# kserve/modelmesh

Hardware: AMD Instinct MI355X
Metric: placement decisions/sec at 100k models x 10k pods; p99 decision latency (higher is better)
Workload: dtype i64; 1 GPU; C3: 100000 models x 10000 pods, 8 load-target decision(s) per model per step = 800000 decisions per launch (SURVEY.md §8d synthetic fleet); streams=4, hw_queues=4, distinct_batches=6, issuers=1, library_submission_threads=0, resident_input_bytes=384000000

## Files before the change

modelmesh_amd/csrc/mmplace.hip:

```cpp
#include <hip/hip_runtime.h>
#include <dlfcn.h>
#include <rccl/rccl.h>
#include <rocprim/device/device_radix_sort.hpp>
#include <chrono>
#include <rocprim/device/device_merge_sort.hpp>
#include <rocprim/device/device_scan.hpp>

#include <algorithm>
#include <atomic>
#include <cstdarg>
#include <cstdio>
#include <cstdlib>
#include <cstring>
#include <map>
#include <memory>
#include <mutex>
#include <shared_mutex>
#include <thread>
#include <new>
#include <string>
#include <unordered_map>
#include <vector>

#include "../../include/mmplace.h"
// ... 23 lines not shown

thread_local std::string g_thread_err;

struct DevBuf {
    void *p = nullptr;
    size_t cap = 0;
    hipError_t ensure(size_t bytes)
    {
        if (bytes <= cap) return hipSuccess;
        if (p) (void)hipFree(p);
        p = nullptr;
        cap = 0;
        size_t want = std::max<size_t>(bytes, 256);
        want = (want + 255) & ~size_t(255);
        hipError_t e = hipMalloc(&p, want);
        if (e == hipSuccess) cap = want;
        return e;
    }
    void release()
    {
        if (p) (void)hipFree(p);
        p = nullptr;
        cap = 0;
    }
    template <class T>
    T *as() const { return reinterpret_cast<T *>(p); }
};

struct SnapBufs {
    DevBuf pods, lru, rem, cnt, rpm, orig, pos_of, elig, elig_nors, pref, has_pref, fullw, ge, pc, ph, nz, heads, bslots, bpm, bwin, bsurv, bpcs;
    DevBuf sel, rk;
    DevBuf amul;
    int32_t amul_w = 0;
    DevBuf memo, memo_cand, memo_rk;
    DevBuf lmemo;
    DevBuf ctpos;
    uint64_t types_gen = 0;
    int32_t n_bslots = 0;
    void release()
    {
        for (DevBuf *b : {&pods, &lru, &rem, &cnt, &rpm, &orig, &pos_of, &elig, &elig_nors, &pref, &has_pref, &fullw, &ge, &pc, &ph, &nz, &heads, &bslots, &bpm, &bwin, &bsurv, &bpcs, &ctpos, &sel, &rk, &amul, &memo, &memo_cand, &memo_rk, &lmemo})
            b->release();
    }
};

template <class SnapT>
SnapT snap_columns(const SnapBufs &B, int32_t P, int32_t W, int32_t T, bool any_rs, int64_t min_space)
{
    SnapT S{};
    S.P = P;
    S.W = W;
    S.T = T;
    S.any_rs = any_rs;
    S.min_space = min_space;
    S.lru = B.lru.as<int64_t>();
    S.rem = B.rem.as<int64_t>();
    S.cnt = B.cnt.as<int32_t>();
    S.rpm = B.rpm.as<int32_t>();
    S.orig = B.orig.as<int32_t>();
    S.pos_of = B.pos_of.as<int32_t>();
    S.elig = B.elig.as<uint64_t>();
    S.elig_nors = B.elig_nors.as<uint64_t>();
    S.pref = B.pref.as<uint64_t>();
    S.has_pref = B.has_pref.as<uint8_t>();
    S.fullw = B.fullw.as<uint64_t>();
    return S;
}

struct SnapSide {
    DevBuf d_allowed, d_has_allowed, stats_acc, d_pts, d_prohib, pstats, tstats, rmodels;
    DevBuf mtw;
    uint64_t types_gen = 0;
    bool rmodels_ok = false;
    std::vector<int32_t> pts_of;
// ... 1733 lines not shown
    HIP_TRY(c, B.elig_nors.ensure((size_t)T * Wc * 8));
    HIP_TRY(c, B.pref.ensure((size_t)T * Wc * 8));
    HIP_TRY(c, B.has_pref.ensure(T));
    HIP_TRY(c, B.fullw.ensure((size_t)Wc * 8));
    HIP_TRY(c, B.ge.ensure((size_t)kGeRows * Wc * 8));
    return MMP_OK;
}
int ensure_commit_scratch(mmp_ctx *c, SnapSide &N, int32_t T, int32_t W)
{
    HIP_TRY(c, c->occupancy.ensure((size_t)W * 64 * 4));
    HIP_TRY(c, c->flag.ensure(sizeof(int32_t)));
    HIP_TRY(c, N.stats_acc.ensure(sizeof(StatsAcc)));
    HIP_TRY(c, c->rs_bad.ensure((size_t)W * 64));
    HIP_TRY(c, c->rs_list.ensure(std::max<size_t>(c->replaced_rs.size(), 1) * 4));
    HIP_TRY(c, N.d_allowed.ensure(std::max<size_t>((size_t)T * W, 1) * 8));
    HIP_TRY(c, c->d_prefer.ensure(std::max<size_t>((size_t)T * W, 1) * 8));
    HIP_TRY(c, N.d_has_allowed.ensure(T));
    return MMP_OK;
}
int ensure_snapshot_buffers(mmp_ctx *c, SnapBufs &B, SnapSide &N, const CommitDims &D)
{
    const int32_t T = D.T, W = D.W;
    HIP_TRY(c, B.pods.ensure(std::max<size_t>(D.P, 1) * sizeof(mmp_pod_row)));
    if (const int rc = ensure_columns(c, B, T, W, W)) return rc;
    HIP_TRY(c, B.ctpos.ensure((size_t)(kGeRows + 1) * 4));
    HIP_TRY(c, B.pc.ensure((size_t)2 * T * (W + 1) * 4));
    HIP_TRY(c, B.nz.ensure((size_t)2 * T * (W + 1) * 4));
    HIP_TRY(c, B.ph.ensure((size_t)2 * T * (W + 1) * 8));
    if (D.have_sel) {
        HIP_TRY(c, B.sel.ensure(D.sel_bytes));
        HIP_TRY(c, B.rk.ensure(D.sel_bytes));
    }
    if (D.have_lmemo) HIP_TRY(c, B.lmemo.ensure((size_t)T * kLongLevels * sizeof(LongMemo)));
    HIP_TRY(c, B.memo.ensure((size_t)kWinLds * sizeof(TypeMemo)));
    HIP_TRY(c, B.memo_cand.ensure((size_t)kWinLds * kMemoCand * 4));
    HIP_TRY(c, B.memo_rk.ensure((size_t)kWinLds * kMemoCand * 2));
    HIP_TRY(c, B.heads.ensure(D.wins_bytes));
    HIP_TRY(c, B.bslots.ensure(kBSlots * sizeof(BSlot) + 16));
    HIP_TRY(c, B.bpm.ensure((size_t)kBSlots * W * 64 * 4));
    HIP_TRY(c, B.bwin.ensure(kBSlots * sizeof(BLaunch)));
    HIP_TRY(c, B.bsurv.ensure((size_t)kBSlots * kBClasses * W * 8));
    HIP_TRY(c, B.bpcs.ensure((size_t)kBSlots * kBClasses * (W + 1) * 4));
    HIP_TRY(c, c->rank.ensure(D.padded * 4));
    return ensure_commit_scratch(c, N, T, W);
}

void clear_commit_scratch(mmp_ctx *c, SnapBufs &B, const CommitDims &D, hipStream_t st)
{
    ZeroBatch zb(st);
    zb.add(c->rank.p, D.padded * 4);
    zb.add(c->occupancy.p, D.padded * 4);
    zb.add(c->flag.p, sizeof(int32_t));
    zb.add(B.bslots.p, kBSlots * sizeof(BSlot) + 16);
    zb.launch(st);
    hipLaunchKernelGGL(zero_tails_kernel, dim3(1), dim3(64), 0, st, B.lru.as<int64_t>(), B.rem.as<int64_t>(), B.cnt.as<int32_t>(),
                       B.rpm.as<int32_t>(), B.orig.as<int32_t>(), B.pos_of.as<int32_t>(), D.P, (int32_t)D.padded);
}

struct OrderCheck {
    bool sort_legal;
    int32_t n_present, n_nonfull;
};
OrderCheck check_placement_order(const std::vector<mmp_pod_row> &pods, int64_t min_space, int64_t churn2)
{
    bool versions_differ = false, full_low_lru = false, wide_count = false;
    OrderCheck oc{};
    for (const mmp_pod_row &r : pods) {
// ... 105 lines not shown
    }
    const size_t n_rs = c->replaced_rs.size();
    if (n_rs) HIP_TRY(c, hipMemcpyAsync(c->rs_list.p, c->replaced_rs.data(), n_rs * 4, hipMemcpyHostToDevice, st));
    in.init = StatsAcc{};
    in.init.global_lru = INT64_MAX;
    HIP_TRY(c, hipMemcpyAsync(N.stats_acc.p, &in.init, sizeof in.init, hipMemcpyHostToDevice, st));
    return MMP_OK;
}

int ensure_audit_multipliers(mmp_ctx *c, SnapBufs &B, int32_t W, hipStream_t st)
{
    if (B.amul_w == W) return MMP_OK;
    HIP_TRY(c, B.amul.ensure((size_t)W * 8));
    std::vector<uint64_t> am((size_t)W);
    for (int32_t w = 0; w < W; w++) am[(size_t)w] = audit_mul((uint64_t)w);
    HIP_TRY(c, hipMemcpyAsync(B.amul.p, am.data(), (size_t)W * 8, hipMemcpyHostToDevice, st));
    HIP_TRY(c, hipStreamSynchronize(st));
    B.amul_w = W;
    return MMP_OK;
}

Snap snap_of(const SnapBufs &B, const CommitDims &D)
{
    Snap S = snap_columns<Snap>(B, D.P, D.W, D.T, D.n_rs > 0, D.min_space);
    S.ge = B.ge.as<uint64_t>();
    S.pc = B.pc.as<int32_t>();
    S.nz = B.nz.as<int32_t>();
    S.ph = B.ph.as<uint64_t>();
    S.ctpos = D.P > 0 ? B.ctpos.as<int32_t>() : nullptr;
    S.amul = B.amul.as<uint64_t>();
    S.sel = D.P > 0 && D.have_sel ? B.sel.as<int32_t>() : nullptr;
    S.rk = D.P > 0 && D.have_sel ? B.rk.as<int32_t>() : nullptr;
    S.memo = B.memo.as<TypeMemo>();
    S.memo_cand = B.memo_cand.as<int32_t>();
    S.memo_rk = B.memo_rk.as<int16_t>();
    S.lmemo = D.have_lmemo ? B.lmemo.as<LongMemo>() : nullptr;
    return S;
}

int launch_rank(mmp_ctx *c, const mmp_pod_row *d_pods, int32_t P, int32_t p_lo, int32_t p_hi, bool slice, bool want_sort, bool sort_legal,
                int32_t *d_rank, hipStream_t st)
{
    const int64_t min_space = c->cfg.min_space_units, churn2 = churn2_of(c);
    if (want_sort && sort_legal && P >= kSampleMinPods && c->tune.rank_mode != 3)
        return rank_by_sampling(c, d_pods, P, min_space, churn2, p_lo, p_hi, d_rank, st);
    if (want_sort && sort_legal && P >= 2) {
        HIP_TRY(c, c->rk_rows.ensure((size_t)P * sizeof(RankRow)));
        HIP_TRY(c, c->rk_idx.ensure((size_t)P * sizeof(RankRow)));
        const PlacementRowLess less{churn2};
        size_t tmp_bytes = 0;
        HIP_TRY(c, rocprim::merge_sort(nullptr, tmp_bytes, c->rk_rows.as<RankRow>(), c->rk_idx.as<RankRow>(), (size_t)P, less, st));
        HIP_TRY(c, c->rk_tmp.ensure(std::max<size_t>(tmp_bytes, 16)));
        hipLaunchKernelGGL(rank_rows_kernel, dim3(div_up(P, 256)), dim3(256), 0, st, d_pods, P, min_space, c->rk_rows.as<RankRow>());
        HIP_TRY(c, rocprim::merge_sort(c->rk_tmp.p, tmp_bytes, c->rk_rows.as<RankRow>(), c->rk_idx.as<RankRow>(), (size_t)P, less, st));
        if (slice)
            hipLaunchKernelGGL(rank_from_order_range_kernel, dim3(div_up(P, 256)), dim3(256), 0, st, c->rk_idx.as<RankRow>(), P, p_lo, p_hi, d_rank);
        else
            hipLaunchKernelGGL(rank_from_order_kernel, dim3(div_up(P, 256)), dim3(256), 0, st, c->rk_idx.as<RankRow>(), P, d_rank);
        return MMP_OK;
    }
    const int pb = div_up(p_hi - p_lo, kRankBlock);
    const int slices = std::max(1, std::min(64, 2048 / pb));
    hipLaunchKernelGGL(rank_pods_kernel, dim3(pb, slices), dim3(kRankBlock), 0, st, d_pods, P, min_space, churn2, slices, p_lo, p_hi, d_rank);
    return MMP_OK;
}

// ... 35 lines not shown
    L1.nb_ge = div_up(kGeRows * W, 4);
    L1.nb_stats = std::min(div_up(P, 256), 512);
    L1.nb_pstats = N.n_pts > 0 ? std::min(div_up(P, 256), 64) : 0;
    return L1;
}
inline int32_t *n_bslots_dev(const SnapBufs &B) { return reinterpret_cast<int32_t *>(static_cast<char *>(B.bslots.p) + kBSlots * sizeof(BSlot)); }
CommitL2 make_commit_l2(const mmp_ctx *c, const SnapBufs &B, const SnapSide &N, const Snap &S)
{
    CommitL2 L2{};
    L2.S = S;
    L2.pods = B.pods.as<mmp_pod_row>();
    L2.wins = B.heads.as<TypeWin>();
    L2.slots = B.bslots.as<BSlot>();
    L2.n_slots = n_bslots_dev(B);
    L2.acc = N.stats_acc.as<StatsAcc>();
    L2.pstats = N.pstats.as<StatsAcc>();
    L2.NP = N.n_pts;
    L2.Tw = N.pts_tw;
    L2.prohib = N.d_prohib.as<uint64_t>();
    L2.has_allowed = c->n_types > 0 ? N.d_has_allowed.as<uint8_t>() : nullptr;
    L2.tstats = N.tstats.as<StatsAcc>();
    L2.nb_finish = div_up(std::max(N.n_pts, S.T), 64);
    return L2;
}
void launch_snapshot_tables(mmp_ctx *c, SnapBufs &B, SnapSide &N, const Snap &S, const CommitDims &D, hipStream_t st)
{
    const int32_t T = D.T, W = D.W;
    const CommitL1 L1 = make_commit_l1(c, B, N, D);
    hipLaunchKernelGGL(commit_level1_kernel, dim3(L1.nb_stats + L1.nb_pstats + 1 + L1.nb_masks + L1.nb_ge), dim3(256), 0, st, L1);
    const CommitL2 L2 = make_commit_l2(c, B, N, S);
    hipLaunchKernelGGL(commit_level2_kernel, dim3(4 * T + L2.nb_finish), dim3(64), 0, st, L2);
    hipLaunchKernelGGL(build_sel_memo_kernel, dim3((D.have_sel ? 2 * T * W : 0) + std::min(T, kWinLds) + (S.lmemo ? T : 0)), dim3(64), 0, st, S,
                       D.have_sel ? B.sel.as<int32_t>() : nullptr, D.have_sel ? B.rk.as<int32_t>() : nullptr, B.heads.as<TypeWin>(),
                       B.memo.as<TypeMemo>(), B.memo_cand.as<int32_t>(), B.memo_rk.as<int16_t>(), B.lmemo.as<LongMemo>());
    hipLaunchKernelGGL(prefix_min_rpm_kernel, dim3(kBSlots), dim3(64), 0, st, S, B.bslots.as<BSlot>(), n_bslots_dev(B), B.bpm.as<int32_t>(),
                       (int32_t)(W * 64));
    hipLaunchKernelGGL(build_bsurv_kernel, dim3(kBSlots), dim3(256), 0, st, S, B.bslots.as<BSlot>(), n_bslots_dev(B), B.bpm.as<int32_t>(),
                       (int32_t)(W * 64), B.bwin.as<BLaunch>(), B.bsurv.as<uint64_t>(), B.bpcs.as<int32_t>());
}
int clear_snapshot_tables(mmp_ctx *c, SnapBufs &B, const CommitDims &D, hipStream_t st)
{
    const size_t T = D.T, W = D.W;
    HIP_TRY(c, hipMemsetAsync(B.heads.p, 0, D.wins_bytes, st));
    HIP_TRY(c, hipMemsetAsync(B.memo.p, 0, (size_t)kWinLds * sizeof(TypeMemo), st));
    HIP_TRY(c, hipMemsetAsync(B.pc.p, 0, 2 * T * (W + 1) * 4, st));
    HIP_TRY(c, hipMemsetAsync(B.nz.p, 0, 2 * T * (W + 1) * 4, st));
    HIP_TRY(c, hipMemsetAsync(B.ph.p, 0, 2 * T * (W + 1) * 8, st));
    HIP_TRY(c, hipMemsetAsync(B.elig.p, 0, T * W * 8, st));
    HIP_TRY(c, hipMemsetAsync(B.elig_nors.p, 0, T * W * 8, st));
    HIP_TRY(c, hipMemsetAsync(B.pref.p, 0, T * W * 8, st));
    HIP_TRY(c, hipMemsetAsync(B.fullw.p, 0, W * 8, st));
    HIP_TRY(c, hipMemsetAsync(B.ge.p, 0, kGeRows * W * 8, st));
    return MMP_OK;
}


int stage_partitions(mmp_ctx *c, SnapSide &N, int32_t P, hipStream_t st)
{
    const int32_t T = std::max(c->n_types, 1), Tw = div_up(T, 64);
    N.pts_of.assign(P, -1);
    N.pts_prohib.clear();
    N.n_pts = 0;
    N.pts_tw = Tw;
    if (c->n_types > 0) {
        if (!c->sig_valid || (int32_t)c->sig_of.size() != P) {
            std::map<std::vector<uint64_t>, int32_t> intern;
            std::vector<uint64_t> sig(Tw);
            const int32_t Wf = c->types_w;
            c->sig_of.assign(P, 0);
            c->sig_rows.clear();
            for (int32_t p = 0; p < P; p++) {
                std::fill(sig.begin(), sig.end(), 0);
                for (int32_t t = 0; t < c->n_types; t++)
                    if (c->has_allowed[t] && !((c->allowed[(size_t)t * Wf + (p >> 6)] >> (p & 63)) & 1ull))
                        sig[t >> 6] |= 1ull << (t & 63);
                auto it = intern.find(sig);
                if (it == intern.end()) {
// ... 161 lines not shown
    return MMP_OK;
} MMP_CATCH(c, "mmp_snapshot_commit")

int mmp_delta_commits(mmp_ctx *c, int64_t *n_out)
{
    if (!c || !n_out) return fail(c, MMP_EINVAL, "mmp_delta_commits: null argument");
    std::lock_guard<std::mutex> gb(c->batch_mu);
    *n_out = c->n_delta_commits;
    return MMP_OK;
}

int mmp_get_order(mmp_ctx *c, int32_t *order_out, int32_t *n_out)
try {
    if (!c || !order_out || !n_out) return fail(c, MMP_EINVAL, "mmp_get_order: null argument");
    std::lock_guard<std::mutex> gb(c->batch_mu);
    std::lock_guard<std::shared_mutex> g(c->mu);
    if (!c->committed) return fail(c, MMP_ESTATE, "no committed snapshot");
    if (c->n_shards > 0) return fail(c, MMP_ESTATE, "mmp_get_order: a pod-axis shard holds only its own slice of the order");
    HIP_TRY(c, hipSetDevice(c->cfg.device));
    const int32_t n = c->stats.instance_count;
    if (n) HIP_TRY(c, copy_sync(c, order_out, c->snap.orig, (size_t)n * 4, hipMemcpyDeviceToHost));
    *n_out = n;
    return MMP_OK;
} MMP_CATCH(c, "mmp_get_order")

int mmp_shortlists(mmp_ctx *c, mmp_shortlist_row *rows, int32_t cap_rows, int32_t *n_rows_out)
try {
    if (!c || !n_rows_out || (!rows && cap_rows > 0) || cap_rows < 0) return fail(c, MMP_EINVAL, "mmp_shortlists: bad argument");
    std::lock_guard<std::mutex> gb(c->batch_mu);
    std::lock_guard<std::shared_mutex> g(c->mu);
    if (!c->committed) return fail(c, MMP_ESTATE, "no committed snapshot");
    HIP_TRY(c, hipSetDevice(c->cfg.device));
    const int32_t nt = c->snap.memo ? std::min(c->snap.T, kWinLds) : 0;
    std::vector<TypeMemo> h((size_t)std::max(nt, 1));
    if (nt) HIP_TRY(c, copy_sync(c, h.data(), c->snap.memo, (size_t)nt * sizeof(TypeMemo), hipMemcpyDeviceToHost));
    for (int32_t i = 0; i < 2 * nt && i < cap_rows; i++) {
        const MemoVar &v = h[i >> 1].v[i & 1];
        rows[i] = mmp_shortlist_row{v.valid, v.lo, v.hi, v.ccount};
    }
    *n_rows_out = 2 * nt;
    return MMP_OK;
} MMP_CATCH(c, "mmp_shortlists")

int mmp_long_shortlists(mmp_ctx *c, mmp_shortlist_row *rows, int32_t cap_rows, int32_t *n_rows_out)
try {
    if (!c || !n_rows_out || (!rows && cap_rows > 0) || cap_rows < 0) return fail(c, MMP_EINVAL, "mmp_long_shortlists: bad argument");
    std::lock_guard<std::mutex> gb(c->batch_mu);
    std::lock_guard<std::shared_mutex> g(c->mu);
    if (!c->committed) return fail(c, MMP_ESTATE, "no committed snapshot");
    HIP_TRY(c, hipSetDevice(c->cfg.device));
    const int32_t nt = c->snap.lmemo ? c->snap.T : 0;
    std::vector<LongMemo> h((size_t)std::max(nt, 1) * kLongLevels);
    if (nt) HIP_TRY(c, copy_sync(c, h.data(), c->snap.lmemo, (size_t)nt * kLongLevels * sizeof(LongMemo), hipMemcpyDeviceToHost));
    for (int32_t i = 0; i < 2 * nt && i < cap_rows; i++) {
        const LongMemo &m = h[(size_t)(i >> 1) * kLongLevels];
        const LongVar &v = m.v[i & 1];
        rows[i] = mmp_shortlist_row{v.valid, m.best0, v.end, v.ccount};
    }
    *n_rows_out = 2 * nt;
    return MMP_OK;
} MMP_CATCH(c, "mmp_long_shortlists")

int mmp_split_batches(mmp_ctx *c, int64_t *n_split_out, int32_t *off_out)
{
    if (!c) return fail(c, MMP_EINVAL, "mmp_split_batches: null context");
    if (n_split_out) *n_split_out = c->n_split.load(std::memory_order_relaxed);
    if (off_out) *off_out = c->split_off.load(std::memory_order_relaxed) ? 1 : 0;
    return MMP_OK;
// ... 3527 lines not shown
```

modelmesh_amd/csrc/place_kernel.hpp:

```cpp
#pragma once
#include "snapshot.hpp"

namespace mmp {

#ifndef MMP_PLACE_WAVES
#define MMP_PLACE_WAVES 4
#endif
constexpr int kPlaceWaves = MMP_PLACE_WAVES;
constexpr int kPlaceBlock = kPlaceWaves * 64;

#ifdef MMP_PHASE_CLOCK
__device__ unsigned int g_phase[4096][16];
#define PHASE_ROW() (((blockIdx.x * (blockDim.x >> 6)) + (threadIdx.x >> 6)) & 4095)
#define PHASE_T0() unsigned long long ph_t_ = __builtin_amdgcn_s_memtime()
#define PHASE(k)                                                                                   \
    do {                                                                                           \
        const unsigned long long t_ = __builtin_amdgcn_s_memtime();                                \
        if (lane_id() == __ffsll((unsigned long long)__ballot(1)) - 1) g_phase[PHASE_ROW()][k] = (unsigned int)(t_ - ph_t_); \
        ph_t_ = t_;                                                                                \
    } while (0)
#define PHASE_COUNT(k, n)                                                                          \
    do {                                                                                           \
        if (lane_id() == __ffsll((unsigned long long)__ballot(1)) - 1) g_phase[PHASE_ROW()][k] += (unsigned int)(n); \
    } while (0)
// ... 60 lines not shown
    int32_t nw;
    uint32_t flags;
    uint64_t E[kWinWords];
    uint64_t Pm[kWinWords];
    uint64_t F[kWinWords];
    uint16_t ct[kGeRows];
    uint16_t pad_[2];
    WinRow rowsE[kWinRows];
    WinRow rowsP[kWinRows];
};
static_assert(sizeof(TypeWin) % 16 == 0, "TypeWin is staged in 16-byte pieces");
static_assert(kGeRows % 2 == 0, "ct + pad_ keep the rows 16-byte aligned");

constexpr int kMemoCand = kWinWords * 64;
constexpr uint32_t kMtwTypeMask = 15u;
constexpr uint32_t kMtwTail = 1u << 4;
constexpr uint32_t kMtwTail1 = 1u << 5;
constexpr int kMtwOffShift = 8;
constexpr uint32_t kMtwOffMask = 511u;
constexpr uint32_t kMtwNone = kMtwTypeMask | kMtwTail | kMtwTail1;
static_assert(kWinLds <= 15 && kMemoCand < 511, "mtw packs a type row in 4 bits and a window offset + 1 in 9");
constexpr int kMtwMaxEnts = 32;
constexpr int kRkNone = -1;
constexpr int kRkFirst = -2;
struct __attribute__((aligned(16))) MemoVar {
    int32_t valid;
    int32_t lo, hi;
    int32_t ccount;
    uint64_t hsum;
    uint32_t hash;
    int32_t pad_;
};
static_assert(sizeof(MemoVar) == 32, "MemoVar is 32 bytes");
struct __attribute__((aligned(16))) TypeMemoHead {
    int64_t b_rem, b_lru;
    int32_t best_is_full, b_rpm, best_idx;
    int32_t plain;
    MemoVar v[2];
    int32_t w0;
    int32_t bestpos, best0;
    int32_t e_rpm;
    int32_t sbk;
    int32_t end0;
    int32_t pad_[2];
};
static_assert(sizeof(TypeMemoHead) == 128, "TypeMemoHead is 128 bytes");
constexpr int kMemoNear = 64;
struct __attribute__((aligned(16))) TypeMemo : TypeMemoHead {
    int32_t cand64[kMemoNear];
    int16_t rk64[kMemoNear];
};
static_assert(sizeof(TypeMemo) == 512, "TypeMemo is 512 bytes");
__host__ __device__ constexpr int memo_stage_bytes(int type_rows)
{
    return (((type_rows < kWinLds ? type_rows : kWinLds) * (int)sizeof(TypeMemo) + 1023) / 1024) * 1024;
}

struct __attribute__((aligned(16))) LongVar {
    int32_t valid;
    int32_t end;
    int32_t ccount;
    int32_t g0;
    uint64_t hsum;
    uint64_t pad_;
};
struct __attribute__((aligned(16))) LongMemo {
    int64_t b_rem, b_lru;
    int32_t best_is_full, b_rpm, best_idx, has_pm;
    int32_t best0, bestpos, e_rpm, sbk;
    LongVar v[2];
    int32_t pad_[4];
};
static_assert(sizeof(LongVar) == 32 && sizeof(LongMemo) == 128, "LongMemo is one 128-byte line");
constexpr int kLongLevels = 3;
struct LongCap {
    int32_t nsb;
    int32_t ok;
    LongMemo m;
};

struct PlaceArgs {
    const mmp_place_req *reqs;
    const mmp_model_row *models;
    const ResolvedModel *rmodels;
    const int32_t *mtw;
    const TypeWin *wins;
    const struct BSlot *bslots;
    const struct BLaunch *bwin;
    const uint64_t *bsurv;
// ... 640 lines not shown
        const mmp_model_row m = A.models[rq.model];
        r.type = (m.type < 0 || m.type >= S.T) ? 0 : m.type;
        const int32_t n_ents = m.n_loaded + m.n_failed;
        r.n_excl = n_ents + rq.n_extra;
        if (r.n_excl <= kInlineExcl) {
#pragma unroll
            for (int i = 0; i < kInlineExcl; i++) {
                if (i < r.n_excl) {
                    const int32_t pod = i < n_ents ? A.ent_pod[m.ent_off + i] : A.extra[rq.extra_off + i - n_ents];
                    r.excl_pos[i] = pod_view_pos<VIEW>(S, pod, P_all);
                }
            }
        }
    }
    return r;
}

__device__ __forceinline__ ResolvedModel resolve_model_row(const Snap &S, const mmp_model_row &m, const int32_t *__restrict__ ent_pod, uint32_t &mtw)
{
    ResolvedModel r;
    r.type = (m.type < 0 || m.type >= S.T) ? 0 : m.type;
    r.n_ents = m.n_loaded + m.n_failed;
#pragma unroll
    for (int k = 0; k < kResolvedInline; k++) {
        int32_t pos = -1;
        if (k < r.n_ents) {
            const int32_t pod = ent_pod[m.ent_off + k];
            if (pod >= 0 && pod < S.P) pos = S.pos_of[pod];
        }
        r.pos[k] = pos;
    }
    mtw = kMtwNone;
    if (S.memo && r.type < kWinLds && r.n_ents <= kMtwMaxEnts) {
        const TypeMemo &M = S.memo[r.type];
        const MemoVar v0 = M.v[0], v1 = M.v[1];
        const int wl = M.w0 * 64;
        const int16_t *RK = S.memo_rk + (size_t)r.type * kMemoCand;
        uint32_t w = (uint32_t)r.type, o1 = 0, o2 = 0;
        for (int k = 0; k < r.n_ents; k++) {
            const int32_t pod = ent_pod[m.ent_off + k];
            if (pod < 0 || pod >= S.P) continue;
            const int32_t pos = S.pos_of[pod];
            if (v0.valid && pos >= v0.lo && pos < v0.hi) {
                const int rk = RK[pos - wl];
                if (rk == 0 || rk == kRkFirst)
                    w |= kMtwTail;
                else if (rk > 0) {
                    const uint32_t off = (uint32_t)(pos - wl) + 1u;
                    if (off == o1 || off == o2) continue;
                    if (!o1)
                        o1 = off;
                    else if (!o2)
                        o2 = off;
                    else
                        w |= kMtwTail;
                }
            }
            if (v1.valid && pos >= v1.lo && pos < v1.hi && (pos == M.best0 || pos == M.bestpos || pos == v1.hi - 1)) w |= kMtwTail1;
        }
        mtw = w | (o1 << kMtwOffShift) | (o2 << (kMtwOffShift + 9));
    }
    return r;
}

__global__ void resolve_models_kernel(Snap S, const mmp_model_row *__restrict__ models,
                                      const int32_t *__restrict__ ent_pod, int32_t n_models,
                                      ResolvedModel *__restrict__ out, int32_t *__restrict__ mtw)
// ... 1196 lines not shown
    __builtin_nontemporal_store(*reinterpret_cast<const v4i_ *>(&o), reinterpret_cast<v4i_ *>(p));
}
template <int FORM>
__device__ __forceinline__ bool memo_try(const Snap &S, const PlaceArgs &A, const mmp_place_req &rq, int d, const TypeMemo *rows)
{
    const bool m_ok = (uint32_t)rq.model < (uint32_t)A.n_models;
    uint32_t mw = (uint32_t)A.mtw[m_ok ? rq.model : 0];
    if (!m_ok) mw = kMtwNone;
    const bool s_ok = (uint32_t)rq.self_pod < (uint32_t)S.P;
    int32_t sp = S.pos_of[s_ok ? rq.self_pod : 0];
    if (!s_ok) sp = -1;
    int32_t xp[kLateExtra];
#pragma unroll
    for (int j = 0; j < kLateExtra; j++) xp[j] = -1;
    const bool x_ok = (uint32_t)rq.n_extra <= (uint32_t)kLateExtra && !(A.extra_bound != 0 && bad_extra_range(A, rq));
    if (__ballot(x_ok && rq.n_extra > 0)) {
        int32_t ep[kLateExtra];
#pragma unroll
        for (int j = 0; j < kLateExtra; j++) {
            const int32_t *pa = (x_ok && j < rq.n_extra) ? A.extra + rq.extra_off + j : S.pos_of;
            ep[j] = *pa;
        }
#pragma unroll
        for (int j = 0; j < kLateExtra; j++) {
            const bool on = x_ok && j < rq.n_extra && (uint32_t)ep[j] < (uint32_t)S.P;
            const int32_t v = S.pos_of[on ? ep[j] : 0];
            xp[j] = on ? v : -1;
        }
    }
    const int type = (int)(mw & kMtwTypeMask);
    const bool t_ok = type < kWinLds && x_ok;
    const TypeMemo *Mp = &rows[type < kWinLds ? type : 0];
    const int64_t b_rem = Mp->b_rem, b_lru = Mp->b_lru;
    const int4 bh = *reinterpret_cast<const int4 *>(&Mp->best_is_full);
    const int4 v0h = *reinterpret_cast<const int4 *>(&Mp->v[0]), v1h = *reinterpret_cast<const int4 *>(&Mp->v[1]);
    const uint64_t hs0 = Mp->v[0].hsum, hs1 = Mp->v[1].hsum;
    const int32_t full = bh.x, b_rpm = bh.y, best_idx = bh.z;
    const int64_t f_rem = remaining_of(rq.fresh_capacity, rq.fresh_used);
    bool nsb = f_rem < S.min_space || f_rem < (b_rem >> 2);
    if (__ballot(full != 0)) {
        const int64_t rel = age_of(b_lru, A.now) / 10;
        const int64_t d1 = jsub64(rq.fresh_lru, b_lru);
        if (full) nsb = d1 > 45000LL && d1 > rel;
    }
    const int4 vh = nsb ? v1h : v0h;
    uint64_t hsum = nsb ? hs1 : hs0;
    const int lo = vh.y;
    const uint32_t len = (uint32_t)(vh.z - lo);
    bool miss = !t_ok || !vh.x || (mw & (nsb ? kMtwTail1 : kMtwTail)) != 0;
    bool x_in = false;
#pragma unroll
    for (int j = 0; j < kLateExtra; j++) x_in |= (uint32_t)(xp[j] - lo) < len;
    const bool sp_in = (uint32_t)(sp - lo) < len;
    const uint32_t moff = nsb ? 0u : (mw >> kMtwOffShift);
    const bool favour = (rq.flags & MMP_REQ_FAVOUR_SELF) != 0;
    int ccount = vh.w;
    int r1 = 0, r2 = 0;
    int ks = 0;
    bool self_in = false, self_best = false;
    int32_t e_rpm = 0;
    const bool own = !miss && (x_in || sp_in || moff != 0);
    if (__ballot(own)) {
        if (own) {
            const int4 mt = *reinterpret_cast<const int4 *>(&Mp->w0);
            const int32_t sbk = Mp->sbk;
            const int wl = mt.x * 64;
            const int16_t *RK = S.memo_rk + type * kMemoCand;
            const int o1 = (int)(moff & kMtwOffMask) - 1, o2 = (int)((moff >> 9) & kMtwOffMask) - 1;
            int qp[kLateExtra + 3];
            qp[0] = sp_in ? sp : -1;
            qp[1] = o1 >= 0 ? wl + o1 : -1;
            qp[2] = o2 >= 0 ? wl + o2 : -1;
#pragma unroll
            for (int j = 0; j < kLateExtra; j++) qp[3 + j] = (uint32_t)(xp[j] - lo) < len ? xp[j] : -1;
            int qr[kLateExtra + 3];
            bool far = false;
#pragma unroll
            for (int j = 0; j < kLateExtra + 3; j++) {
                const int rel = qp[j] - lo;
                const bool near = qp[j] >= 0 && rel < kMemoNear;
                qr[j] = (int)Mp->rk64[near ? rel : 0];
                if (!near) qr[j] = kRkNone;
                far |= qp[j] >= 0 && rel >= kMemoNear;
            }
            if (__ballot(far)) {
#pragma unroll
                for (int j = 0; j < kLateExtra + 3; j++) {
                    const bool f = qp[j] >= 0 && qp[j] - lo >= kMemoNear;
                    int g = (int)RK[f ? qp[j] - wl : 0];
                    asm volatile("" : "+v"(g));
                    if (f) qr[j] = g;
                }
            }
            const int srk = qr[0], m1 = qr[1], m2 = qr[2];
            int xr[kLateExtra];
#pragma unroll
            for (int j = 0; j < kLateExtra; j++) xr[j] = qr[3 + j];
            const int end_v = vh.z - 1;
            auto take = [&](int rk, int pos) {
                if (rk == 0 || rk == kRkFirst || (nsb && pos == end_v))
                    miss = true;
                else if (!nsb && rk > 0 && rk != r1 && rk != r2) {
                    if (r1 == 0)
                        r1 = rk;
                    else if (r2 == 0)
                        r2 = rk;
                    else
                        miss = true;
                    hsum -= audit_mul((uint64_t)(pos >> 6)) << (pos & 63);
                }
            };
            take(m1, wl + o1);
            take(m2, wl + o2);
#pragma unroll
            for (int j = 0; j < kLateExtra; j++) take(xr[j], xp[j]);
            if (sp_in) {
                if (srk == 0) {
                    if (favour)
                        self_best = true;
                    else
                        miss = true;
                } else if (srk == kRkFirst)
                    miss = true;
                else if (nsb) {
                    if (sp == end_v) miss = true;
                } else if (srk > 0 && srk != r1 && srk != r2) {
                    if (sbk)
                        miss = true;
                    else {
                        self_in = true;
                        ks = srk;
                        e_rpm = mt.w;
                    }
                }
            }
            ccount -= (r1 != 0) + (r2 != 0);
        }
    }
    if (miss) return false;
    mmp_place_out o;
    o.best = best_idx;
    if (self_best || (self_in && favour)) {
        o.chosen = MMP_SELF;
        o.n_candidates = 0;
        o.hash = 0;
        store_out_streaming(A.outs + d, o);
        return true;
    }
    const int32_t f_rpm = rq.fresh_rpm;
    const int n_others = ccount - 1 - (self_in ? 1 : 0);
    int32_t mn = b_rpm;
    if (self_in && e_rpm < mn) mn = e_rpm;
    if (n_others > 0 && f_rpm < mn) mn = f_rpm;
    RpmRule rule;
    rule.init(age_of(rq.last_used, A.now), mn);
    const int32_t lim = rule.limit();
    const bool null0 = ccount >= 2 && b_rpm >= 100 && b_rpm > lim;
    const bool null_s = ccount >= 2 && self_in && e_rpm >= 100 && e_rpm > lim;
    const bool null_o = ccount >= 2 && n_others > 0 && f_rpm >= 100 && f_rpm > lim;
    const int remaining = ccount - (null0 ? 1 : 0) - (null_s ? 1 : 0) - (null_o ? n_others : 0);
    const int index = remaining <= 1 ? 0 : (int)(((uint64_t)rq.pick * (uint64_t)(uint32_t)remaining) >> 32);
    int k;
    if (null_o)
        k = (!null0 && index == 0) ? 0 : ks;
    else {
        k = index + (null0 ? 1 : 0);
        if (__ballot(null_s || r1 != 0)) {
            int a = null_s ? ks : INT32_MAX, b = r1 ? r1 : INT32_MAX, c = r2 ? r2 : INT32_MAX, t;
            if (a > b) { t = a; a = b; b = t; }
            if (b > c) { t = b; b = c; c = t; }
            if (a > b) { t = a; a = b; b = t; }
            if (a <= k) k++;
            if (b <= k) k++;
            if (c <= k) k++;
        }
    }
    o.chosen = MMP_NONE;
    if (remaining >= 1) {
        o.chosen = Mp->cand64[k < kMemoNear ? k : 0];
        if (k >= kMemoNear) {
            int32_t g = S.memo_cand[type * kMemoCand + k];
            asm volatile("" : "+v"(g));
            o.chosen = g;
        }
        if (k == 0) o.chosen = best_idx;
        if (self_in && k == ks) o.chosen = MMP_SELF;
    }
    o.n_candidates = ccount;
    o.hash = (uint32_t)(hsum ^ (hsum >> 32)) ^ ((uint32_t)remaining * 0x9E3779B1u);
    store_out_streaming(A.outs + d, o);
    return true;
}

__device__ __forceinline__ bool long_memo_try(const Snap &S, const PlaceArgs &A, const ResolvedReq &r, mmp_place_out &o)
{
    bool miss = r.type < 0 || r.n_excl > kInlineExcl || A.force_wave;
#ifdef MMP_PHASE_CLOCK
    if (miss) PHASE_WHY(1);
#endif
    const LongMemo *Mp = S.lmemo + (size_t)(r.type < 0 ? 0 : r.type) * kLongLevels;
    int64_t b_rem = Mp->b_rem, b_lru = Mp->b_lru;
    int4 h1 = *reinterpret_cast<const int4 *>(&Mp->best_is_full);
    int4 h2 = *reinterpret_cast<const int4 *>(&Mp->best0);
    int4 v0 = *reinterpret_cast<const int4 *>(&Mp->v[0]), v1 = *reinterpret_cast<const int4 *>(&Mp->v[1]);
    uint64_t hs0 = Mp->v[0].hsum, hs1 = Mp->v[1].hsum;
    const int32_t nb1 = Mp[1].best0;
    auto excluded = [&](int p) {
        bool x = false;
#pragma unroll
        for (int i = 0; i < kInlineExcl; i++) x |= r.excl_pos[i] == p;
        return x;
    };
    int lvl = 0;
// ... 375 lines not shown

#ifndef MMP_PLACE_EU
#define MMP_PLACE_EU 6
#endif
__global__ __launch_bounds__(kPlaceBlock) __attribute__((amdgpu_waves_per_eu(MMP_PLACE_EU, MMP_PLACE_EU))) void place_batch_kernel(Snap S, PlaceArgs A, int32_t wpad)
{
    extern __shared__ __attribute__((aligned(16))) unsigned char smem[];
    place_block<false>(S, A, wpad, smem);
}

__global__ __launch_bounds__(kPlaceBlock) void place_batch_long_kernel(Snap S, PlaceArgs A, int32_t wpad)
{
    extern __shared__ __attribute__((aligned(16))) unsigned char smem[];
    place_block<true, kReq64, false, true>(S, A, wpad, smem);
}

constexpr int kLongDenseFrom = 3 * 4 * 256 * 64;
__global__ __launch_bounds__(kPlaceBlock) __attribute__((amdgpu_waves_per_eu(4, 4))) void place_batch_long4_kernel(Snap S, PlaceArgs A, int32_t wpad)
{
    extern __shared__ __attribute__((aligned(16))) unsigned char smem[];
    place_block<true>(S, A, wpad, smem);
}

#ifndef MMP_C_WAVES
#define MMP_C_WAVES 7
#endif
__global__ __launch_bounds__(kPlaceBlock) __attribute__((amdgpu_waves_per_eu(MMP_C_WAVES, MMP_C_WAVES))) void place_batch_c_kernel(Snap S, PlaceArgs A, int32_t wpad,
                                                                                                            mmp_place_caller C)
{
    extern __shared__ __attribute__((aligned(16))) unsigned char smem[];
    place_block<false, kReqC>(S, A, wpad, smem, nullptr, C);
}
__device__ __forceinline__ void build_memo_body(int t, const Snap &S, const TypeWin *__restrict__ wins, TypeMemo *__restrict__ memo,
                                                int32_t *__restrict__ cand, int16_t *__restrict__ rkt)
{
    constexpr int kScr = 2;
    __shared__ uint64_t scr[kWinWords * kScr];
    __shared__ MemoCap caps[2];
    __shared__ int ok[2];
    const int lane = lane_id();
    if (lane < 2) {
        PlaceArgs A{};
        ResolvedReq r{};
        r.type = t;
        r.selfpos = -1;
        r.n_late = -1;
#pragma unroll
        for (int i = 0; i < kInlineExcl; i++) r.excl_pos[i] = -1;
#pragma unroll
        for (int i = 0; i < kLateExtra; i++) r.late_pos[i] = -1;
        MemoCap mc{};
        mc.nsb = lane;
        mmp_place_out o;
        const int code = lane_decide_win<false, true, kScr>(S, A, r, wins, scr + lane, o, &mc);
        caps[lane] = mc;
        ok[lane] = code == kLaneDone && mc.ccount <= kMemoCand;
    }
    __syncthreads();
    const int w0 = wins[t].w0;
    const bool any = ok[0] || ok[1];
    const MemoCap &c0 = caps[ok[0] ? 0 : 1];
    if (lane == 0) {
        TypeMemoHead M{};
        M.b_rem = c0.b_rem;
        M.b_lru = c0.b_lru;
        M.best_is_full = c0.best_is_full;
        M.b_rpm = c0.b_rpm;
        M.best_idx = c0.best_idx;
        M.plain = c0.bestpos == c0.best0;
        M.w0 = w0;
        M.bestpos = c0.bestpos;
        M.best0 = c0.best0;
        M.e_rpm = c0.e_rpm;
        M.sbk = c0.sbk ? 1 : 0;
        M.end0 = caps[0].end;
        for (int v = 0; v < 2; v++) {
            const MemoCap &c = caps[v];
            M.v[v].valid = ok[v];
            M.v[v].lo = c.best0;
            M.v[v].hi = c.end == kNoPos ? S.P : c.end + 1;
            M.v[v].ccount = c.ccount;
            M.v[v].hsum = c.hsum;
            M.v[v].hash = (uint32_t)(c.hsum ^ (c.hsum >> 32));
        }
        static_cast<TypeMemoHead &>(memo[t]) = M;
    }
    __shared__ int32_t near_c[kMemoNear];
    __shared__ int32_t near_r[kMemoNear];
    near_c[lane] = 0;
    near_r[lane] = kRkNone;
    wave_sync();
    int32_t *out = cand + (size_t)t * kMemoCand;
    int16_t *rk = rkt + (size_t)t * kMemoCand;
    int running = 0;
    for (int j = 0; j < kWinWords; j++) {
        const int w = w0 + j, pos = w * 64 + lane;
        const uint64_t word = (ok[0] && w >= caps[0].wlo && w <= caps[0].whi) ? scr[j * kScr] : 0ull;
        const bool bit = (word >> lane) & 1ull;
        const int k = running + __popcll((unsigned long long)(word & ((1ull << lane) - 1ull)));
        int v = kRkNone;
        if (bit) {
            v = k;
            const int32_t pod = S.orig[pos];
            out[k] = pod;
            if (k < kMemoNear) near_c[k] = pod;
        }
        if (any && pos == c0.bestpos) v = 0;
        if (any && pos == c0.best0 && c0.best0 != c0.bestpos) v = kRkFirst;
        rk[j * 64 + lane] = (int16_t)v;
        if (any && pos >= c0.best0 && pos - c0.best0 < kMemoNear) near_r[pos - c0.best0] = v;
        running += __popcll((unsigned long long)word);
    }
    wave_sync();
    memo[t].cand64[lane] = near_c[lane];
    memo[t].rk64[lane] = (int16_t)near_r[lane];
}
__global__ __launch_bounds__(64) void build_sel_memo_kernel(Snap S, int32_t *__restrict__ sel, int32_t *__restrict__ rk, const TypeWin *__restrict__ wins,
                                                            TypeMemo *__restrict__ memo, int32_t *__restrict__ cand, int16_t *__restrict__ memo_rk,
                                                            LongMemo *__restrict__ lmemo)
{
    const int n_sel = sel ? 2 * S.T * S.W : 0;
    const int n_memo = S.T < kWinLds ? S.T : kWinLds;
    if ((int)blockIdx.x < n_sel)
        build_sel_body((int)blockIdx.x, S, sel, rk);
    else if ((int)blockIdx.x < n_sel + n_memo)
        build_memo_body((int)blockIdx.x - n_sel, S, wins, memo, cand, memo_rk);
    else
        build_long_memo_body((int)blockIdx.x - n_sel - n_memo, S, lmemo);
}

__global__ __launch_bounds__(kPlaceBlock) __attribute__((amdgpu_waves_per_eu(MMP_C_WAVES, MMP_C_WAVES))) void place_batch_c_m_kernel(Snap S, PlaceArgs A, int32_t wpad,
                                                                                                              mmp_place_caller C)
{
    extern __shared__ __attribute__((aligned(16))) unsigned char smem[];
    place_block<false, kReqC, true, true>(S, A, wpad, smem, nullptr, C);
}
__global__ __launch_bounds__(kPlaceBlock) __attribute__((amdgpu_waves_per_eu(7, 7))) void place_batch_m_kernel(Snap S, PlaceArgs A, int32_t wpad)
{
    extern __shared__ __attribute__((aligned(16))) unsigned char smem[];
    place_block<false, kReq64, true, true>(S, A, wpad, smem);
}
constexpr int kMemoFrom = 4 * 1024 * 64;
constexpr int kMemoFromC = 3 * 1024 * 64;
constexpr int kSplitFrom = 6 * 1024 * 64;
constexpr int kSplitFromC = 8 * 1024 * 64;

constexpr int kRestLists = 64;
constexpr int kRestCntStride = 32;
__host__ __device__ constexpr int rest_list_cap(int n_words) { return ((n_words + kRestLists - 1) / kRestLists) * 64; }
__host__ __device__ constexpr size_t rest_buffer_ints(int n_words) { return (size_t)kRestLists * kRestCntStride + (size_t)kRestLists * rest_list_cap(n_words); }

__device__ __forceinline__ void rest_append(int32_t *__restrict__ rest, int32_t cap, int d, bool todo)
{
    const uint64_t mk = __ballot(todo);
    if (mk && rest) {
        const int l = __builtin_amdgcn_readfirstlane(d >> 6) & (kRestLists - 1);
        const int first = __ffsll((unsigned long long)mk) - 1;
        int base = 0;
        if (lane_id() == first)
// ... 235 lines not shown
```

modelmesh_amd/csrc/snapshot.hpp:

```cpp
#pragma once
#include <hip/hip_runtime.h>
#include <stdint.h>

#include "../../include/mmplace.h"
#include "wave.hpp"

namespace mmp {

struct Snap {
    int32_t P;
    int32_t W;
    int32_t T;
    int32_t any_rs;
    int64_t min_space;
    const int64_t *lru;
    const int64_t *rem;
    const int32_t *cnt;
    const int32_t *rpm;
    const int32_t *orig;
    const int32_t *pos_of;
    const uint64_t *elig;
    const uint64_t *elig_nors;
    const uint64_t *pref;
    const uint8_t *has_pref;
    const uint64_t *fullw;
    const uint64_t *ge;
    int32_t pos_base;
    int32_t w_base;
    int32_t more_after;
    const int32_t *pc;
    const uint64_t *ph;
    const int32_t *nz;
    const int32_t *ctpos;
    const int32_t *sel;
    const int32_t *rk;
    const uint64_t *amul;
    const struct TypeMemo *memo;
    const int32_t *memo_cand;
    const int16_t *memo_rk;
    const struct LongMemo *lmemo;
};

constexpr int kGeBase = 10;
constexpr int kGeRows = 54;

struct __attribute__((aligned(16))) RankRow {
    int64_t vers, rem, lru, cap;
    int32_t count, lt_free, lip, rpm;
    uint32_t id_order, flags;
    uint32_t pad0, pad1;
};
static_assert(sizeof(RankRow) == 64, "RankRow is 64 bytes");

__device__ __forceinline__ int64_t jsub64(int64_t a, int64_t b) { return (int64_t)((uint64_t)a - (uint64_t)b); }
__device__ __forceinline__ int64_t age_of(int64_t t, int64_t now) { return t == 0 ? 0 : jsub64(now, t); }

__host__ __device__ __forceinline__ int64_t remaining_of(int64_t cap, int64_t used)
{
    int64_t d = (int64_t)((uint64_t)cap - (uint64_t)used);
    return d > 0 ? d : 0;
}

__host__ __device__ __forceinline__ RankRow make_rank_row(const mmp_pod_row &r, int64_t min_space)
{
    RankRow o;
    o.vers = r.version;
    o.rem = remaining_of(r.capacity, r.used);
    o.lru = r.lru_time;
    o.cap = r.capacity;
    o.count = r.count;
// ... 481 lines not shown
```

Baseline: 49.46 billion decisions/s.

## Split type memo into compact hot row and separate cold table

Splits the 512-byte per-type memo into a 256-byte hot row read by the placement fast path and a 128-byte cold table holding the full variant records used elsewhere. The hot row packs flags, bounds and counts into fewer words, stores candidates as 16-bit and ranks as 8-bit. Entries that do not fit fall back to the global candidate array or mark the memo invalid. The goal is to halve the LDS staging and memory traffic per type row and allow more rows to be resident, at the cost of extra branches and possible memo misses when candidates exceed 16 bits or ranks exceed 127.

```diff
diff --git a/modelmesh_amd/csrc/mmplace.hip b/modelmesh_amd/csrc/mmplace.hip
--- a/modelmesh_amd/csrc/mmplace.hip
+++ b/modelmesh_amd/csrc/mmplace.hip
@@ -79,14 +79,14 @@
     DevBuf sel, rk;
     DevBuf amul;
     int32_t amul_w = 0;
-    DevBuf memo, memo_cand, memo_rk;
+    DevBuf memo, memo_cold, memo_cand, memo_rk;
     DevBuf lmemo;
     DevBuf ctpos;
     uint64_t types_gen = 0;
     int32_t n_bslots = 0;
     void release()
     {
-        for (DevBuf *b : {&pods, &lru, &rem, &cnt, &rpm, &orig, &pos_of, &elig, &elig_nors, &pref, &has_pref, &fullw, &ge, &pc, &ph, &nz, &heads, &bslots, &bpm, &bwin, &bsurv, &bpcs, &ctpos, &sel, &rk, &amul, &memo, &memo_cand, &memo_rk, &lmemo})
+        for (DevBuf *b : {&pods, &lru, &rem, &cnt, &rpm, &orig, &pos_of, &elig, &elig_nors, &pref, &has_pref, &fullw, &ge, &pc, &ph, &nz, &heads, &bslots, &bpm, &bwin, &bsurv, &bpcs, &ctpos, &sel, &rk, &amul, &memo, &memo_cold, &memo_cand, &memo_rk, &lmemo})
             b->release();
     }
 };
@@ -1886,7 +1886,8 @@
         HIP_TRY(c, B.rk.ensure(D.sel_bytes));
     }
     if (D.have_lmemo) HIP_TRY(c, B.lmemo.ensure((size_t)T * kLongLevels * sizeof(LongMemo)));
-    HIP_TRY(c, B.memo.ensure((size_t)kWinLds * sizeof(TypeMemo)));
+    HIP_TRY(c, B.memo.ensure(kMemoTableBytes));
+    HIP_TRY(c, B.memo_cold.ensure((size_t)kWinLds * sizeof(TypeMemoCold)));
     HIP_TRY(c, B.memo_cand.ensure((size_t)kWinLds * kMemoCand * 4));
     HIP_TRY(c, B.memo_rk.ensure((size_t)kWinLds * kMemoCand * 2));
     HIP_TRY(c, B.heads.ensure(D.wins_bytes));
@@ -2058,6 +2059,7 @@
     S.sel = D.P > 0 && D.have_sel ? B.sel.as<int32_t>() : nullptr;
     S.rk = D.P > 0 && D.have_sel ? B.rk.as<int32_t>() : nullptr;
     S.memo = B.memo.as<TypeMemo>();
+    S.memo_cold = B.memo_cold.as<TypeMemoCold>();
     S.memo_cand = B.memo_cand.as<int32_t>();
     S.memo_rk = B.memo_rk.as<int16_t>();
     S.lmemo = D.have_lmemo ? B.lmemo.as<LongMemo>() : nullptr;
@@ -2159,7 +2161,7 @@
     hipLaunchKernelGGL(commit_level2_kernel, dim3(4 * T + L2.nb_finish), dim3(64), 0, st, L2);
     hipLaunchKernelGGL(build_sel_memo_kernel, dim3((D.have_sel ? 2 * T * W : 0) + std::min(T, kWinLds) + (S.lmemo ? T : 0)), dim3(64), 0, st, S,
                        D.have_sel ? B.sel.as<int32_t>() : nullptr, D.have_sel ? B.rk.as<int32_t>() : nullptr, B.heads.as<TypeWin>(),
-                       B.memo.as<TypeMemo>(), B.memo_cand.as<int32_t>(), B.memo_rk.as<int16_t>(), B.lmemo.as<LongMemo>());
+                       B.memo.as<TypeMemo>(), B.memo_cold.as<TypeMemoCold>(), B.memo_cand.as<int32_t>(), B.memo_rk.as<int16_t>(), B.lmemo.as<LongMemo>());
     hipLaunchKernelGGL(prefix_min_rpm_kernel, dim3(kBSlots), dim3(64), 0, st, S, B.bslots.as<BSlot>(), n_bslots_dev(B), B.bpm.as<int32_t>(),
                        (int32_t)(W * 64));
     hipLaunchKernelGGL(build_bsurv_kernel, dim3(kBSlots), dim3(256), 0, st, S, B.bslots.as<BSlot>(), n_bslots_dev(B), B.bpm.as<int32_t>(),
@@ -2169,7 +2171,8 @@
 {
     const size_t T = D.T, W = D.W;
     HIP_TRY(c, hipMemsetAsync(B.heads.p, 0, D.wins_bytes, st));
-    HIP_TRY(c, hipMemsetAsync(B.memo.p, 0, (size_t)kWinLds * sizeof(TypeMemo), st));
+    HIP_TRY(c, hipMemsetAsync(B.memo.p, 0, kMemoTableBytes, st));
+    HIP_TRY(c, hipMemsetAsync(B.memo_cold.p, 0, (size_t)kWinLds * sizeof(TypeMemoCold), st));
     HIP_TRY(c, hipMemsetAsync(B.pc.p, 0, 2 * T * (W + 1) * 4, st));
     HIP_TRY(c, hipMemsetAsync(B.nz.p, 0, 2 * T * (W + 1) * 4, st));
     HIP_TRY(c, hipMemsetAsync(B.ph.p, 0, 2 * T * (W + 1) * 8, st));
@@ -2397,8 +2400,8 @@
     if (!c->committed) return fail(c, MMP_ESTATE, "no committed snapshot");
     HIP_TRY(c, hipSetDevice(c->cfg.device));
     const int32_t nt = c->snap.memo ? std::min(c->snap.T, kWinLds) : 0;
-    std::vector<TypeMemo> h((size_t)std::max(nt, 1));
-    if (nt) HIP_TRY(c, copy_sync(c, h.data(), c->snap.memo, (size_t)nt * sizeof(TypeMemo), hipMemcpyDeviceToHost));
+    std::vector<TypeMemoCold> h((size_t)std::max(nt, 1));
+    if (nt) HIP_TRY(c, copy_sync(c, h.data(), c->snap.memo_cold, (size_t)nt * sizeof(TypeMemoCold), hipMemcpyDeviceToHost));
     for (int32_t i = 0; i < 2 * nt && i < cap_rows; i++) {
         const MemoVar &v = h[i >> 1].v[i & 1];
         rows[i] = mmp_shortlist_row{v.valid, v.lo, v.hi, v.ccount};
diff --git a/modelmesh_amd/csrc/place_kernel.hpp b/modelmesh_amd/csrc/place_kernel.hpp
--- a/modelmesh_amd/csrc/place_kernel.hpp
+++ b/modelmesh_amd/csrc/place_kernel.hpp
@@ -116,7 +116,7 @@
     int32_t pad_;
 };
 static_assert(sizeof(MemoVar) == 32, "MemoVar is 32 bytes");
-struct __attribute__((aligned(16))) TypeMemoHead {
+struct __attribute__((aligned(16))) TypeMemoCold {
     int64_t b_rem, b_lru;
     int32_t best_is_full, b_rpm, best_idx;
     int32_t plain;
@@ -128,17 +128,31 @@
     int32_t end0;
     int32_t pad_[2];
 };
-static_assert(sizeof(TypeMemoHead) == 128, "TypeMemoHead is 128 bytes");
+static_assert(sizeof(TypeMemoCold) == 128, "TypeMemoCold is 128 bytes");
 constexpr int kMemoNear = 64;
-struct __attribute__((aligned(16))) TypeMemo : TypeMemoHead {
-    int32_t cand64[kMemoNear];
-    int16_t rk64[kMemoNear];
+constexpr uint32_t kMemoFull = 1u;
+constexpr uint32_t kMemoSbk = 2u;
+constexpr uint32_t kMemoValid0 = 4u;
+constexpr uint32_t kMemoValid1 = 8u;
+constexpr int kMemoHeadShift = 8;
+struct __attribute__((aligned(16))) TypeMemo {
+    int64_t b_rem, b_lru;
+    uint32_t flags;
+    int32_t b_rpm, best_idx, e_rpm;
+    int32_t lo, hi0, hi1;
+    uint32_t ccounts;
+    uint64_t hsum0, hsum1;
+    uint16_t cand16[kMemoNear];
+    int8_t rk8[kMemoNear];
 };
-static_assert(sizeof(TypeMemo) == 512, "TypeMemo is 512 bytes");
+static_assert(sizeof(TypeMemo) == 256, "TypeMemo is 256 bytes");
+static_assert((sizeof(TypeMemo) & (sizeof(TypeMemo) - 1)) == 0, "a hot row is a power of two");
+static_assert(kMemoCand < 65536 && kMemoNear <= 127, "ccounts packs two counts in 16 bits each; rk8 holds candidate numbers below kMemoNear");
 __host__ __device__ constexpr int memo_stage_bytes(int type_rows)
 {
     return (((type_rows < kWinLds ? type_rows : kWinLds) * (int)sizeof(TypeMemo) + 1023) / 1024) * 1024;
 }
+constexpr size_t kMemoTableBytes = (size_t)memo_stage_bytes(kWinLds);
 
 struct __attribute__((aligned(16))) LongVar {
     int32_t valid;
@@ -845,7 +859,7 @@
     }
     mtw = kMtwNone;
     if (S.memo && r.type < kWinLds && r.n_ents <= kMtwMaxEnts) {
-        const TypeMemo &M = S.memo[r.type];
+        const TypeMemoCold &M = S.memo_cold[r.type];
         const MemoVar v0 = M.v[0], v1 = M.v[1];
         const int wl = M.w0 * 64;
         const int16_t *RK = S.memo_rk + (size_t)r.type * kMemoCand;
@@ -2108,10 +2122,11 @@
     const bool t_ok = type < kWinLds && x_ok;
     const TypeMemo *Mp = &rows[type < kWinLds ? type : 0];
     const int64_t b_rem = Mp->b_rem, b_lru = Mp->b_lru;
-    const int4 bh = *reinterpret_cast<const int4 *>(&Mp->best_is_full);
-    const int4 v0h = *reinterpret_cast<const int4 *>(&Mp->v[0]), v1h = *reinterpret_cast<const int4 *>(&Mp->v[1]);
-    const uint64_t hs0 = Mp->v[0].hsum, hs1 = Mp->v[1].hsum;
-    const int32_t full = bh.x, b_rpm = bh.y, best_idx = bh.z;
+    const int4 bh = *reinterpret_cast<const int4 *>(&Mp->flags);
+    const int4 lh = *reinterpret_cast<const int4 *>(&Mp->lo);
+    const uint64_t hs0 = Mp->hsum0, hs1 = Mp->hsum1;
+    const uint32_t mflags = (uint32_t)bh.x;
+    const int32_t full = (int32_t)(mflags & kMemoFull), b_rpm = bh.y, best_idx = bh.z;
     const int64_t f_rem = remaining_of(rq.fresh_capacity, rq.fresh_used);
     bool nsb = f_rem < S.min_space || f_rem < (b_rem >> 2);
     if (__ballot(full != 0)) {
@@ -2119,18 +2134,17 @@
         const int64_t d1 = jsub64(rq.fresh_lru, b_lru);
         if (full) nsb = d1 > 45000LL && d1 > rel;
     }
-    const int4 vh = nsb ? v1h : v0h;
     uint64_t hsum = nsb ? hs1 : hs0;
-    const int lo = vh.y;
-    const uint32_t len = (uint32_t)(vh.z - lo);
-    bool miss = !t_ok || !vh.x || (mw & (nsb ? kMtwTail1 : kMtwTail)) != 0;
+    const int lo = lh.x, hi = nsb ? lh.z : lh.y;
+    const uint32_t len = (uint32_t)(hi - lo);
+    bool miss = !t_ok || !(mflags & (nsb ? kMemoValid1 : kMemoValid0)) || (mw & (nsb ? kMtwTail1 : kMtwTail)) != 0;
     bool x_in = false;
 #pragma unroll
     for (int j = 0; j < kLateExtra; j++) x_in |= (uint32_t)(xp[j] - lo) < len;
     const bool sp_in = (uint32_t)(sp - lo) < len;
     const uint32_t moff = nsb ? 0u : (mw >> kMtwOffShift);
     const bool favour = (rq.flags & MMP_REQ_FAVOUR_SELF) != 0;
-    int ccount = vh.w;
+    int ccount = (int)(nsb ? (uint32_t)lh.w >> 16 : (uint32_t)lh.w & 0xffffu);
     int r1 = 0, r2 = 0;
     int ks = 0;
     bool self_in = false, self_best = false;
@@ -2138,9 +2152,8 @@
     const bool own = !miss && (x_in || sp_in || moff != 0);
     if (__ballot(own)) {
         if (own) {
-            const int4 mt = *reinterpret_cast<const int4 *>(&Mp->w0);
-            const int32_t sbk = Mp->sbk;
-            const int wl = mt.x * 64;
+            const bool sbk = (mflags & kMemoSbk) != 0;
+            const int wl = lo & ~63;
             const int16_t *RK = S.memo_rk + type * kMemoCand;
             const int o1 = (int)(moff & kMtwOffMask) - 1, o2 = (int)((moff >> 9) & kMtwOffMask) - 1;
             int qp[kLateExtra + 3];
@@ -2155,7 +2168,7 @@
             for (int j = 0; j < kLateExtra + 3; j++) {
                 const int rel = qp[j] - lo;
                 const bool near = qp[j] >= 0 && rel < kMemoNear;
-                qr[j] = (int)Mp->rk64[near ? rel : 0];
+                qr[j] = (int)Mp->rk8[near ? rel : 0];
                 if (!near) qr[j] = kRkNone;
                 far |= qp[j] >= 0 && rel >= kMemoNear;
             }
@@ -2172,7 +2185,7 @@
             int xr[kLateExtra];
 #pragma unroll
             for (int j = 0; j < kLateExtra; j++) xr[j] = qr[3 + j];
-            const int end_v = vh.z - 1;
+            const int end_v = hi - 1;
             auto take = [&](int rk, int pos) {
                 if (rk == 0 || rk == kRkFirst || (nsb && pos == end_v))
                     miss = true;
@@ -2206,7 +2219,7 @@
                     else {
                         self_in = true;
                         ks = srk;
-                        e_rpm = mt.w;
+                        e_rpm = bh.w;
                     }
                 }
             }
@@ -2253,8 +2266,9 @@
     }
     o.chosen = MMP_NONE;
     if (remaining >= 1) {
-        o.chosen = Mp->cand64[k < kMemoNear ? k : 0];
-        if (k >= kMemoNear) {
+        const int n_head = (int)((mflags >> kMemoHeadShift) & 0xffu);
+        o.chosen = (int32_t)Mp->cand16[k < n_head ? k : 0];
+        if (k >= n_head) {
             int32_t g = S.memo_cand[type * kMemoCand + k];
             asm volatile("" : "+v"(g));
             o.chosen = g;
@@ -2696,7 +2710,7 @@
     place_block<false, kReqC>(S, A, wpad, smem, nullptr, C);
 }
 __device__ __forceinline__ void build_memo_body(int t, const Snap &S, const TypeWin *__restrict__ wins, TypeMemo *__restrict__ memo,
-                                                int32_t *__restrict__ cand, int16_t *__restrict__ rkt)
+                                                TypeMemoCold *__restrict__ cold, int32_t *__restrict__ cand, int16_t *__restrict__ rkt)
 {
     constexpr int kScr = 2;
     __shared__ uint64_t scr[kWinWords * kScr];
@@ -2718,14 +2732,14 @@
         mmp_place_out o;
         const int code = lane_decide_win<false, true, kScr>(S, A, r, wins, scr + lane, o, &mc);
         caps[lane] = mc;
-        ok[lane] = code == kLaneDone && mc.ccount <= kMemoCand;
+        ok[lane] = code == kLaneDone && mc.ccount <= kMemoCand && (mc.best0 >> 6) == wins[t].w0;
     }
     __syncthreads();
     const int w0 = wins[t].w0;
     const bool any = ok[0] || ok[1];
     const MemoCap &c0 = caps[ok[0] ? 0 : 1];
     if (lane == 0) {
-        TypeMemoHead M{};
+        TypeMemoCold M{};
         M.b_rem = c0.b_rem;
         M.b_lru = c0.b_lru;
         M.best_is_full = c0.best_is_full;
@@ -2747,7 +2761,7 @@
             M.v[v].hsum = c.hsum;
             M.v[v].hash = (uint32_t)(c.hsum ^ (c.hsum >> 32));
         }
-        static_cast<TypeMemoHead &>(memo[t]) = M;
+        cold[t] = M;
     }
     __shared__ int32_t near_c[kMemoNear];
     __shared__ int32_t near_r[kMemoNear];
@@ -2776,11 +2790,32 @@
         running += __popcll((unsigned long long)word);
     }
     wave_sync();
-    memo[t].cand64[lane] = near_c[lane];
-    memo[t].rk64[lane] = (int16_t)near_r[lane];
+    const int32_t pc = near_c[lane], pr = near_r[lane];
+    const uint64_t wide = __ballot((uint32_t)pc > 0xffffu);
+    const int n_head = wide ? __ffsll((unsigned long long)wide) - 1 : kMemoNear;
+    const bool fits = __ballot(pr > 127) == 0;
+    memo[t].cand16[lane] = (uint16_t)(lane < n_head ? pc : 0);
+    memo[t].rk8[lane] = (int8_t)(fits ? pr : kRkNone);
+    if (lane == 0) {
+        TypeMemo &H = memo[t];
+        H.b_rem = c0.b_rem;
+        H.b_lru = c0.b_lru;
+        H.flags = (c0.best_is_full ? kMemoFull : 0u) | (c0.sbk ? kMemoSbk : 0u) | (ok[0] && fits ? kMemoValid0 : 0u) |
+                  (ok[1] && fits ? kMemoValid1 : 0u) | ((uint32_t)n_head << kMemoHeadShift);
+        H.b_rpm = c0.b_rpm;
+        H.best_idx = c0.best_idx;
+        H.e_rpm = c0.e_rpm;
+        H.lo = c0.best0;
+        H.hi0 = caps[0].end == kNoPos ? S.P : caps[0].end + 1;
+        H.hi1 = caps[1].end == kNoPos ? S.P : caps[1].end + 1;
+        H.ccounts = ((uint32_t)caps[0].ccount & 0xffffu) | ((uint32_t)caps[1].ccount << 16);
+        H.hsum0 = caps[0].hsum;
+        H.hsum1 = caps[1].hsum;
+    }
 }
 __global__ __launch_bounds__(64) void build_sel_memo_kernel(Snap S, int32_t *__restrict__ sel, int32_t *__restrict__ rk, const TypeWin *__restrict__ wins,
-                                                            TypeMemo *__restrict__ memo, int32_t *__restrict__ cand, int16_t *__restrict__ memo_rk,
+                                                            TypeMemo *__restrict__ memo, TypeMemoCold *__restrict__ memo_cold, int32_t *__restrict__ cand,
+                                                            int16_t *__restrict__ memo_rk,
                                                             LongMemo *__restrict__ lmemo)
 {
     const int n_sel = sel ? 2 * S.T * S.W : 0;
@@ -2788,7 +2823,7 @@
     if ((int)blockIdx.x < n_sel)
         build_sel_body((int)blockIdx.x, S, sel, rk);
     else if ((int)blockIdx.x < n_sel + n_memo)
-        build_memo_body((int)blockIdx.x - n_sel, S, wins, memo, cand, memo_rk);
+        build_memo_body((int)blockIdx.x - n_sel, S, wins, memo, memo_cold, cand, memo_rk);
     else
         build_long_memo_body((int)blockIdx.x - n_sel - n_memo, S, lmemo);
 }
diff --git a/modelmesh_amd/csrc/snapshot.hpp b/modelmesh_amd/csrc/snapshot.hpp
--- a/modelmesh_amd/csrc/snapshot.hpp
+++ b/modelmesh_amd/csrc/snapshot.hpp
@@ -36,6 +36,7 @@
     const int32_t *rk;
     const uint64_t *amul;
     const struct TypeMemo *memo;
+    const struct TypeMemoCold *memo_cold;
     const int32_t *memo_cand;
     const int16_t *memo_rk;
     const struct LongMemo *lmemo;
```

After: 49.23 billion decisions/s. About the same (-0.5%).
